# arpg/vicalib

Measured on NVIDIA H100. Metric: lm_iterations_per_sec, higher is better.
Workload: dtype f64

## Files before the change

### vicalib_b200/csrc/vc_imu_math.cuh

```cuda
#pragma once
#include "vc_math.cuh"

namespace vc {
namespace imu {

struct D1 {
  double a, v;
  __host__ __device__ D1() : a(0.0), v(0.0) {}
  __host__ __device__ D1(double s) : a(s), v(0.0) {}
  __host__ __device__ D1(double s, double d) : a(s), v(d) {}
};
__device__ __forceinline__ D1 operator+(D1 x, D1 y) { return {x.a + y.a, x.v + y.v}; }
__device__ __forceinline__ D1 operator-(D1 x, D1 y) { return {x.a - y.a, x.v - y.v}; }
__device__ __forceinline__ D1 operator-(D1 x) { return {-x.a, -x.v}; }
__device__ __forceinline__ D1 operator*(D1 x, D1 y) { return {x.a * y.a, x.a * y.v + x.v * y.a}; }
__device__ __forceinline__ D1 operator/(D1 x, D1 y) {
  const double inv = 1.0 / y.a, q = x.a * inv;
  return {q, (x.v - q * y.v) * inv};
}
__device__ __forceinline__ D1 dsqrt(D1 x) { const double s = sqrt(x.a); return {s, 0.5 * x.v / s}; }
__device__ __forceinline__ double dsqrt(double x) { return sqrt(x); }
__device__ __forceinline__ void dsincos(D1 x, D1* s, D1* c) {
  double sn, cs;
  sincos(x.a, &sn, &cs);
  *s = {sn, cs * x.v};
  *c = {cs, -sn * x.v};
}
__device__ __forceinline__ void dsincos(double x, double* s, double* c) { sincos(x, s, c); }
__device__ __forceinline__ D1 dtan(D1 x) { const double t = tan(x.a); return {t, (1.0 + t * t) * x.v}; }
__device__ __forceinline__ double dtan(double x) { return tan(x); }
__device__ __forceinline__ D1 datan(D1 x) { return {atan(x.a), x.v / (1.0 + x.a * x.a)}; }
__device__ __forceinline__ double datan(double x) { return atan(x); }
__device__ __forceinline__ double val(D1 x) { return x.a; }
__device__ __forceinline__ double val(double x) { return x; }

template <class T> struct Vec { T x, y, z; };
template <class T> struct Quat { T x, y, z, w; };

template <class T> __device__ __forceinline__ Vec<T> operator+(Vec<T> a, Vec<T> b) { return {a.x + b.x, a.y + b.y, a.z + b.z}; }
template <class T> __device__ __forceinline__ Vec<T> operator-(Vec<T> a, Vec<T> b) { return {a.x - b.x, a.y - b.y, a.z - b.z}; }
template <class T> __device__ __forceinline__ Vec<T> scale(Vec<T> a, T s) { return {a.x * s, a.y * s, a.z * s}; }
template <class T> __device__ __forceinline__ Vec<T> cross(Vec<T> a, Vec<T> b) {
  return {a.y * b.z - a.z * b.y, a.z * b.x - a.x * b.z, a.x * b.y - a.y * b.x};
}
template <class T> __device__ __forceinline__ T dot(Vec<T> a, Vec<T> b) { return a.x * b.x + a.y * b.y + a.z * b.z; }

template <class T> __device__ __forceinline__ Quat<T> qmul(Quat<T> a, Quat<T> b) {
  return {a.w * b.x + a.x * b.w + a.y * b.z - a.z * b.y, a.w * b.y + a.y * b.w + a.z * b.x - a.x * b.z,
          a.w * b.z + a.z * b.w + a.x * b.y - a.y * b.x, a.w * b.w - a.x * b.x - a.y * b.y - a.z * b.z};
}
template <class T> __device__ __forceinline__ Quat<T> qconj(Quat<T> q) { return {-q.x, -q.y, -q.z, q.w}; }
template <class T> __device__ __forceinline__ Vec<T> qrot(Quat<T> q, Vec<T> v) {
  const Vec<T> qv{q.x, q.y, q.z};
  Vec<T> uv = cross(qv, v);
  uv = uv + uv;
  return v + scale(uv, q.w) + cross(qv, uv);
}

template <class T> __device__ inline Quat<T> so3_exp(Vec<T> om) {
  const T th2 = dot(om, om);
  T imag, real;
  if (val(th2) < 1e-3) {
    imag = T(0.5) + th2 * (T(-1.0 / 48.0) + th2 * (T(1.0 / 3840.0) + th2 * (T(-1.0 / 645120.0) + th2 * T(1.0 / 185794560.0))));
    real = T(1.0) + th2 * (T(-1.0 / 8.0) + th2 * (T(1.0 / 384.0) + th2 * (T(-1.0 / 46080.0) + th2 * (T(1.0 / 10321920.0) +
                                                                                                   th2 * T(-1.0 / 3715891200.0)))));
  } else {
    const T th = dsqrt(th2);
    T s, c;
    dsincos(th * T(0.5), &s, &c);
    imag = s / th;
    real = c;
  }
  return {imag * om.x, imag * om.y, imag * om.z, real};
}
template <class T> __device__ inline Vec<T> so3_log(Quat<T> q, T* theta) {
  const T n2 = q.x * q.x + q.y * q.y + q.z * q.z;
  T f, n = T(0.0);
  if (val(n2) < kSophusEps * kSophusEps) {
    f = T(2.0) / q.w - T(2.0) * n2 / (q.w * q.w * q.w);
    if (val(n2) > 0.0) n = dsqrt(n2);
  } else {
    n = dsqrt(n2);
    if (fabs(val(q.w)) < kSophusEps) f = T(val(q.w) > 0.0 ? M_PI : -M_PI) / n;
    else f = T(2.0) * datan(n / q.w) / n;
  }
  *theta = f * n;
  return {f * q.x, f * q.y, f * q.z};
}
template <class T> __device__ inline void se3_log(Quat<T> q, Vec<T> t, T out[6]) {
  T th;
  const Vec<T> om = so3_log(q, &th);
  T c;
  if (fabs(val(th)) < kSophusEps) c = T(1.0 / 12.0);
  else c = (T(1.0) - th / (T(2.0) * dtan(th * T(0.5)))) / (th * th);
  const Vec<T> ot = cross(om, t);
  const Vec<T> oot = cross(om, ot);
  const Vec<T> u = t - scale(ot, T(0.5)) + scale(oot, c);
  out[0] = u.x; out[1] = u.y; out[2] = u.z;
  out[3] = om.x; out[4] = om.y; out[5] = om.z;
}

struct ImuBuf {
  const double* d;
  int n;
  double start_time, end_time, average_dt;
};
template <class T> struct Meas { Vec<T> w, a; T time; };

template <class T> __device__ __forceinline__ Meas<T> load_meas(const ImuBuf& b, int i) {
  const int64_t n = b.n;
  return {{T(b.d[n + i]), T(b.d[2 * n + i]), T(b.d[3 * n + i])},
          {T(b.d[4 * n + i]), T(b.d[5 * n + i]), T(b.d[6 * n + i])}, T(b.d[i])};
}
template <class T> __device__ inline Meas<T> interpolate(const ImuBuf& b, int ai, int bi, T ts, double time) {
  const Meas<T> ma = load_meas<T>(b, ai), mb = load_meas<T>(b, bi);
  const T t_a = ma.time + ts, t_b = mb.time + ts, t_out = T(time);
  const T fr = (t_out - t_a) / (t_b - t_a), omf = T(1.0) - fr;
  return {scale(ma.w, omf) + scale(mb.w, fr), scale(ma.a, omf) + scale(mb.a, fr), t_out};
}
template <class T> __device__ inline Meas<T> get_element(const ImuBuf& b, double time, T ts, int* idx) {
  const double off = val(ts);
  const int n = b.n;
  double gd = (time - b.start_time + off) / b.average_dt;
  if (!(gd > 0.0)) gd = 0.0;
  int guess = gd >= static_cast<double>(n) ? n - 1 : static_cast<int>(gd);
  guess = min(guess, n - 1);
  Meas<T> r;
  if (b.d[guess] + off > time) {
    if (guess == 0) {
      r = load_meas<T>(b, 0);
      r.time = r.time + ts;
      *idx = 0;
    } else {
      while ((guess - 1) > 0 && b.d[guess - 1] + off > time) --guess;
      r = interpolate<T>(b, guess - 1, guess, ts, time);
      *idx = guess - 1;
    }
  } else {
    if (guess == n - 1) {
      *idx = guess;
      r = load_meas<T>(b, n - 1);
      r.time = r.time + ts;
    } else {
      while ((guess + 1) < n && (b.d[guess + 1] + off) < time) ++guess;
      r = interpolate<T>(b, guess, guess + 1, ts, time);
      *idx = guess;
    }
  }
  return r;
}
template <class T> __device__ inline bool get_next(const ImuBuf& b, double max_time, T ts, int* idx, Meas<T>* out) {
  if (*idx + 1 >= b.n || b.d[*idx + 1] + val(ts) > max_time) {
    *out = get_element<T>(b, max_time, ts, idx);
    return false;
  }
  *out = load_meas<T>(b, ++*idx);
  out->time = out->time + ts;
  return true;
}

template <class T> struct Pose { Vec<T> p; Quat<T> q; Vec<T> v; };

template <class T> __device__ inline Pose<T> integrate_pose(const Pose<T>& y0, const T k[9], T dt) {
  const Quat<T> dq = so3_exp(Vec<T>{k[3] * dt, k[4] * dt, k[5] * dt});
  Pose<T> y;
  y.p = y0.p + Vec<T>{k[0] * dt, k[1] * dt, k[2] * dt};
  y.q = qmul(dq, y0.q);
  y.v = y0.v + Vec<T>{k[6] * dt, k[7] * dt, k[8] * dt};
  return y;
}
template <class T> __device__ inline void pose_derivative(const Pose<T>& y, Vec<T> g, const Meas<T>& z0, const Meas<T>& z1,
                                                          Vec<T> bg, Vec<T> ba, const T sf[6], T dt, T k[9]) {
  const T alpha = (z1.time - (z0.time + dt)) / (z1.time - z0.time), oma = T(1.0) - alpha;
  const Vec<T> zg = scale(z0.w, alpha) + scale(z1.w, oma);
  const Vec<T> za = scale(z0.a, alpha) + scale(z1.a, oma);
  k[0] = y.v.x; k[1] = y.v.y; k[2] = y.v.z;
  const Vec<T> w = qrot(y.q, Vec<T>{zg.x * sf[0] + bg.x, zg.y * sf[1] + bg.y, zg.z * sf[2] + bg.z});
  k[3] = w.x; k[4] = w.y; k[5] = w.z;
  const Vec<T> a = qrot(y.q, Vec<T>{za.x * sf[3] + ba.x, za.y * sf[4] + ba.y, za.z * sf[5] + ba.z}) - g;
  k[6] = a.x; k[7] = a.y; k[8] = a.z;
}
template <class T> __device__ inline Pose<T> integrate_imu(const Pose<T>& y0, const Meas<T>& z0, const Meas<T>& z1, Vec<T> bg,
                                                           Vec<T> ba, const T sf[6], Vec<T> g) {
  if (val(z1.time) == val(z0.time)) return y0;
  const T dt = z1.time - z0.time;
  T k1[9], k2[9], k3[9], k4[9];
  pose_derivative(y0, g, z0, z1, bg, ba, sf, T(0.0), k1);
  const Pose<T> y1 = integrate_pose(y0, k1, dt * T(0.5));
  pose_derivative(y1, g, z0, z1, bg, ba, sf, dt / T(2.0), k2);
  const Pose<T> y2 = integrate_pose(y0, k2, dt * T(0.5));
  pose_derivative(y2, g, z0, z1, bg, ba, sf, dt / T(2.0), k3);
  const Pose<T> y3 = integrate_pose(y0, k3, dt);
  pose_derivative(y3, g, z0, z1, bg, ba, sf, dt, k4);
#pragma unroll
  for (int i = 0; i < 9; ++i) k1[i] = k1[i] + T(2.0) * k2[i] + T(2.0) * k3[i] + k4[i];
  return integrate_pose(y0, k1, dt / T(6.0));
}

template <class T> __device__ inline Vec<T> gravity_vector(T p, T q) {
  T sp, cp, sq, cq;
  dsincos(p, &sp, &cp);
  dsincos(q, &sq, &cq);
  const T mg = T(-9.8007);
  return {cp * sq * mg, -sp * mg, cp * cq * mg};
}

template <class T>
__device__ inline bool imu_raw_residual(const ImuBuf& buf, double t_start, double t_end, const T x2[7], const T x1[7],
                                        const T v2[3], const T v1[3], const T g2[2], const T b[6], const T sf[6], T ts,
                                        T r[9], Pose<T>* end = nullptr) {
  if (!(t_start >= buf.start_time + val(ts) && t_start <= buf.end_time + val(ts)) || buf.n == 0) return false;
  const Vec<T> g = gravity_vector<T>(g2[0], g2[1]);
  const Vec<T> bg{b[0], b[1], b[2]}, ba{b[3], b[4], b[5]};
  Pose<T> y{{x1[4], x1[5], x1[6]}, {x1[0], x1[1], x1[2], x1[3]}, {v1[0], v1[1], v1[2]}};
  int idx;
  Meas<T> prev = get_element<T>(buf, t_start, ts, &idx), cur;
  bool more = true;
  while (more) {
    more = get_next<T>(buf, t_end, ts, &idx, &cur);
    y = integrate_imu(y, prev, cur, bg, ba, sf, g);
    prev = cur;
  }
  if (end) *end = y;
  const Quat<T> q2i = qconj(Quat<T>{x2[0], x2[1], x2[2], x2[3]});
  const Vec<T> t2i = qrot(q2i, Vec<T>{x2[4], x2[5], x2[6]});
  const Quat<T> qe = qmul(y.q, q2i);
  const Vec<T> te = y.p - qrot(y.q, t2i);
  se3_log(qe, te, r);
  r[6] = y.v.x - v2[0];
  r[7] = y.v.y - v2[1];
  r[8] = y.v.z - v2[2];
  return true;
}

}
}
```

### vicalib_b200/csrc/vc_imu_weights.cuh

```cuda
#pragma once
#include "vc_imu_math.cuh"
#include "vc_internal.h"

namespace vc {
namespace wts {

using imu::Meas;
using imu::Pose;
using imu::Quat;
using imu::Vec;

__device__ inline double powi(double x, int y) {
  double r = x;
  for (int i = 1; i < y; ++i) r *= x;
  return r;
}

__device__ inline void dqx_dq(Quat<double> q, Vec<double> v, double* o, int ld) {
  const double x = v.x, y = v.y, z = v.z;
  const double s1 = 2 * q.x * y, s2 = 2 * q.y * y, s3 = 2 * q.x * x, s4 = 2 * q.z * x, s5 = 2 * q.y * z, s6 = 2 * q.z * z;
  o[0] = s2 + s6; o[1] = s1 - 4 * q.y * x + 2 * q.w * z; o[2] = 2 * q.x * z - 2 * q.w * y - 4 * q.z * x; o[3] = s5 - 2 * q.z * y;
  o[ld + 0] = 2 * q.y * x - 4 * q.x * y - 2 * q.w * z; o[ld + 1] = s3 + s6; o[ld + 2] = s5 + 2 * q.w * x - 4 * q.z * y; o[ld + 3] = s4 - 2 * q.x * z;
  o[2 * ld + 0] = s4 + 2 * q.w * y - 4 * q.x * z; o[2 * ld + 1] = 2 * q.z * y - 2 * q.w * x - 4 * q.y * z; o[2 * ld + 2] = s2 + s3; o[2 * ld + 3] = s1 - 2 * q.y * x;
}
__device__ inline void dq1q2_dq2(Quat<double> q1, double* o, int ld) {
  o[0] = q1.w; o[1] = -q1.z; o[2] = q1.y; o[3] = q1.x;
  o[ld] = q1.z; o[ld + 1] = q1.w; o[ld + 2] = -q1.x; o[ld + 3] = q1.y;
  o[2 * ld] = -q1.y; o[2 * ld + 1] = q1.x; o[2 * ld + 2] = q1.w; o[2 * ld + 3] = q1.z;
  o[3 * ld] = -q1.x; o[3 * ld + 1] = -q1.y; o[3 * ld + 2] = -q1.z; o[3 * ld + 3] = q1.w;
}
__device__ inline void dq1q2_dq1(Quat<double> q2, double* o, int ld) {
  o[0] = q2.w; o[1] = q2.z; o[2] = -q2.y; o[3] = q2.x;
  o[ld] = -q2.z; o[ld + 1] = q2.w; o[ld + 2] = q2.x; o[ld + 3] = q2.y;
  o[2 * ld] = q2.y; o[2 * ld + 1] = -q2.x; o[2 * ld + 2] = q2.w; o[2 * ld + 3] = q2.z;
  o[3 * ld] = -q2.x; o[3 * ld + 1] = -q2.y; o[3 * ld + 2] = -q2.z; o[3 * ld + 3] = q2.w;
}
__device__ inline void dqExp_dw(Vec<double> w, double o[12]) {
  const double t = sqrt(w.x * w.x + w.y * w.y + w.z * w.z);
  const double s1 = t / 20 - 1, s2 = powi(t, 2) / 48 - 0.5;
  const double s3 = (s1 * w.y * w.z) / 24, s4 = (s1 * w.x * w.z) / 24, s5 = (s1 * w.x * w.y) / 24, s6 = powi(t, 2);
  o[0] = (s1 * powi(w.x, 2)) / 24 - s6 / 48 + 0.5; o[1] = s5; o[2] = s4;
  o[3] = s5; o[4] = (s1 * powi(w.y, 2)) / 24 - s6 / 48 + 0.5; o[5] = s3;
  o[6] = s4; o[7] = s3; o[8] = (s1 * powi(w.z, 2)) / 24 - s6 / 48 + 0.5;
  o[9] = (s2 * w.x) / 2; o[10] = (s2 * w.y) / 2; o[11] = (s2 * w.z) / 2;
}
__device__ inline void dLog_dq(Quat<double> q, double o[12]) {
  const double x = q.x, y = q.y, z = q.z, w = q.w;
  const double vsq = powi(x, 2) + powi(y, 2) + powi(z, 2), vn = sqrt(vsq);
  if (vn < 1e-9) {
    const double s1 = 2 * vsq, s2 = 1.0 / powi(w, 3), s3 = (3 * s1) / powi(w, 4) - 2 / powi(w, 2), s4 = 2 / w;
    o[0] = -4 * s2 * powi(x, 2) + s4 - s1 * s2; o[1] = -4 * x * y * s2; o[2] = -4 * x * z * s2; o[3] = x * s3;
    o[4] = -4 * x * y * s2; o[5] = -4 * s2 * powi(y, 2) + s4 - s1 * s2; o[6] = -4 * y * z * s2; o[7] = y * s3;
    o[8] = -4 * x * z * s2; o[9] = -4 * y * z * s2; o[10] = -4 * s2 * powi(z, 2) + s4 - s1 * s2; o[11] = z * s3;
  } else {
    const double s1 = vsq, s2 = 1 / (s1 / powi(w, 2) + 1), s3 = atan(sqrt(s1) / w), s4 = 1 / pow(s1, 1.5), s5 = 1 / s1,
                 s6 = 1 / w, s7 = (2 * s3) / sqrt(s1);
    const double s8 = 2 * y * z * s2 * s5 * s6 - 2 * y * z * s3 * s4;
    const double s9 = 2 * x * z * s2 * s5 * s6 - 2 * x * z * s3 * s4;
    const double s10 = 2 * x * y * s2 * s5 * s6 - 2 * x * y * s3 * s4;
    o[0] = s7 - 2 * powi(x, 2) * s3 * s4 + 2 * powi(x, 2) * s2 * s5 * s6; o[1] = s10; o[2] = s9; o[3] = -(2 * x * s2) / powi(w, 2);
    o[4] = s10; o[5] = s7 - 2 * powi(y, 2) * s3 * s4 + 2 * powi(y, 2) * s2 * s5 * s6; o[6] = s8; o[7] = -(2 * y * s2) / powi(w, 2);
    o[8] = s9; o[9] = s8; o[10] = s7 - 2 * powi(z, 2) * s3 * s4 + 2 * powi(z, 2) * s2 * s5 * s6; o[11] = -(2 * z * s2) / powi(w, 2);
  }
}

__device__ inline void dLog_dSE3(Quat<double> q, Vec<double> tr, double dlog[42]) {
  double dw_dq[12];
  dLog_dq(q, dw_dq);
  const double x = tr.x, y = tr.y, z = tr.z;
  double theta;
  const Vec<double> w = imu::so3_log<double>(q, &theta);
  const double wx = w.x, wy = w.y, wz = w.z;
  const bool close_to_zero = fabs(theta) < kSophusEps;
  const double O[9] = {0, -wz, wy, wz, 0, -wx, -wy, wx, 0};
  double O2[9];
  for (int i = 0; i < 3; ++i)
    for (int j = 0; j < 3; ++j) {
      double s = 0;
      for (int k = 0; k < 3; ++k) s += O[i * 3 + k] * O[k * 3 + j];
      O2[i * 3 + j] = s;
    }
  const double cc = close_to_zero ? 1. / 12. : (1.0 - theta / (2.0 * tan(theta / 2.0))) / (theta * theta);
  for (int i = 0; i < 42; ++i) dlog[i] = 0.0;
  for (int i = 0; i < 3; ++i)
    for (int j = 0; j < 3; ++j) dlog[i * 7 + j] = (i == j ? 1.0 : 0.0) - 0.5 * O[i * 3 + j] + cc * O2[i * 3 + j];
  for (int i = 0; i < 3; ++i)
    for (int j = 0; j < 4; ++j) dlog[(3 + i) * 7 + 3 + j] = dw_dq[i * 4 + j];
  double d[9];
  if (close_to_zero) {
    const double div_12 = 1. / 12, div_6 = 1. / 6.;
    const double wx_x = wx * x, wy_x = wy * x, wz_x = wz * x, wx_y = wx * y, wy_y = wy * y, wz_y = wz * y, wx_z = wx * z,
                 wy_z = wy * z, wz_z = wz * z;
    d[0] = div_12 * (wy_y + wz_z); d[1] = div_12 * wx_y - div_6 * wy_x - 0.5 * z; d[2] = 0.5 * y - div_6 * wz_x + div_12 * wx_z;
    d[3] = 0.5 * z + div_12 * wy_x - div_6 * wx_y; d[4] = div_12 * (wx_x + wz_z); d[5] = div_12 * wy_z - div_6 * wz_y - 0.5 * x;
    d[6] = div_12 * wz_x - div_6 * wx_z - 0.5 * y; d[7] = 0.5 * x + div_12 * wz_y - div_6 * wy_z; d[8] = div_12 * (wx_x * wy_y);
  } else {
    const double s1 = powi(wx, 2) + powi(wy, 2) + powi(wz, 2);
    const double s2 = tan(sqrt(s1) / 2);
    const double s3 = sqrt(s1) / (2 * s2) - 1;
    const double s4 = wz / (2 * sqrt(s1) * s2) - (wz * (powi(s2, 2) + 1)) / (4 * powi(s2, 2));
    const double s5 = wy / (2 * sqrt(s1) * s2) - (wy * (powi(s2, 2) + 1)) / (4 * powi(s2, 2));
    const double s6 = wx / (2 * sqrt(s1) * s2) - (wx * (powi(s2, 2) + 1)) / (4 * powi(s2, 2));
    const double s7 = 1 / s1, s8 = 1 / powi(s1, 2);
    const double s9 = powi(wx, 2) + powi(wy, 2), s10 = powi(wx, 2) + powi(wz, 2), s11 = powi(wy, 2) + powi(wz, 2);
    const double s12 = 2 * s3 * s8 * wx * wy * wz;
    const double s13 = -2 * s3 * s8 * wy * powi(wz, 2) + s4 * s7 * wy * wz + s3 * s7 * wy;
    const double s14 = -2 * s3 * s8 * wx * powi(wz, 2) + s4 * s7 * wx * wz + s3 * s7 * wx;
    const double s15 = -2 * s3 * s8 * wz * powi(wy, 2) + s5 * s7 * wz * wy + s3 * s7 * wz;
    const double s16 = -2 * s3 * s8 * wz * powi(wx, 2) + s6 * s7 * wz * wx + s3 * s7 * wz;
    const double s17 = -2 * s3 * s8 * wx * powi(wy, 2) + s5 * s7 * wx * wy + s3 * s7 * wx;
    const double s18 = -2 * s3 * s8 * wy * powi(wx, 2) + s6 * s7 * wy * wx + s3 * s7 * wy;
    const double s19 = 2 * s3 * s7 * wy, s20 = 2 * s3 * s7 * wx;
    d[0] = x * (s6 * s7 * s11 - 2 * s3 * s8 * s11 * wx) - s18 * y - s16 * z;
    d[1] = x * (s19 + s5 * s7 * s11 - 2 * s3 * s8 * s11 * wy) - s17 * y - z * (s5 * s7 * wx * wz - 2 * s3 * s8 * wx * wy * wz + 0.5);
    d[2] = x * (s4 * s7 * s11 + 2 * s3 * s7 * wz - 2 * s3 * s8 * s11 * wz) - s14 * z + y * (s12 - s4 * s7 * wx * wy + 0.5);
    d[3] = y * (s20 + s6 * s7 * s10 - 2 * s3 * s8 * s10 * wx) - s18 * x + z * (s12 - s6 * s7 * wy * wz + 0.5);
    d[4] = y * (s5 * s7 * s10 - 2 * s3 * s8 * s10 * wy) - s17 * x - s15 * z;
    d[5] = y * (s4 * s7 * s10 + 2 * s3 * s7 * wz - 2 * s3 * s8 * s10 * wz) - s13 * z - x * (s4 * s7 * wx * wy - s12 + 0.5);
    d[6] = z * (s20 + s6 * s7 * s9 - 2 * s3 * s8 * s9 * wx) - s16 * x - y * (s6 * s7 * wy * wz - s12 + 0.5);
    d[7] = z * (s19 + s5 * s7 * s9 - 2 * s3 * s8 * s9 * wy) - s15 * y + x * (s12 - s5 * s7 * wx * wz + 0.5);
    d[8] = z * (s4 * s7 * s9 - 2 * s3 * s8 * s9 * wz) - s14 * x - s13 * y;
  }
  for (int i = 0; i < 3; ++i)
    for (int j = 0; j < 4; ++j) {
      double s = 0;
      for (int k = 0; k < 3; ++k) s += d[i * 3 + k] * dw_dq[k * 4 + j];
      dlog[i * 7 + 3 + j] = s;
    }
}

constexpr int kTeam = 16;
struct Work {
  double C[100], A[100], Gm[60], t1[100], t2[100];
  double rot[8];
  int rpq[8];
};

__device__ __forceinline__ void tmm(double* out, const double* A, const double* B, int R, int K, int C, int tl,
                                    bool transB = false) {
  for (int e = tl; e < R * C; e += kTeam) {
    const int r = e / C, c = e - r * C;
    double s = 0.0;
    for (int k = 0; k < K; ++k) s += A[r * K + k] * (transB ? B[c * K + k] : B[k * C + c]);
    out[e] = s;
  }
}

struct StageJac {
  double R[9];
  double Dw[12];
  double Da[12];
};
__device__ __forceinline__ void stage_jac(const Pose<double>& y, const Meas<double>& z0, const Meas<double>& z1, Vec<double> bg,
                                          Vec<double> ba, double dt, StageJac* J) {
  const double alpha = (z1.time - (z0.time + dt)) / (z1.time - z0.time);
  const Vec<double> zg = imu::scale(z0.w, alpha) + imu::scale(z1.w, 1.0 - alpha);
  const Vec<double> za = imu::scale(z0.a, alpha) + imu::scale(z1.a, 1.0 - alpha);
  qmat(Q4{y.q.x, y.q.y, y.q.z, y.q.w}, J->R);
  dqx_dq(y.q, zg + bg, J->Dw, 4);
  dqx_dq(y.q, za + ba, J->Da, 4);
}
__device__ __forceinline__ void stage_T(const double col[10], int j, const StageJac& J, double T[9]) {
  T[0] = col[7]; T[1] = col[8]; T[2] = col[9];
#pragma unroll
  for (int i = 0; i < 3; ++i) {
    T[3 + i] = J.Dw[i * 4] * col[3] + J.Dw[i * 4 + 1] * col[4] + J.Dw[i * 4 + 2] * col[5] + J.Dw[i * 4 + 3] * col[6];
    T[6 + i] = J.Da[i * 4] * col[3] + J.Da[i * 4 + 1] * col[4] + J.Da[i * 4 + 2] * col[5] + J.Da[i * 4 + 3] * col[6];
  }
  const double sel_g = (j >= 10 && j < 13) ? 1.0 : 0.0, sel_a = j >= 13 ? 1.0 : 0.0;
  const int bc = j >= 13 ? j - 13 : (j >= 10 ? j - 10 : 0);
#pragma unroll
  for (int i = 0; i < 3; ++i) {
    const double rv = bc == 0 ? J.R[i * 3] : (bc == 1 ? J.R[i * 3 + 1] : J.R[i * 3 + 2]);
    T[3 + i] += sel_g * rv;
    T[6 + i] += sel_a * rv;
  }
}
__device__ __forceinline__ Pose<double> integrate_push(const Pose<double>& y0, const double k[9], double h, const double T[9], int j,
                                                       double col[10]) {
  const Vec<double> wdt{k[3] * h, k[4] * h, k[5] * h};
  const Quat<double> r = imu::so3_exp<double>(wdt);
  double a[16], e[12];
  dq1q2_dq1(y0.q, a, 4);
  dqExp_dw(wdt, e);
#pragma unroll
  for (int i = 0; i < 3; ++i) {
    col[i] = h * T[i] + (j == i ? 1.0 : 0.0);
    col[7 + i] = h * T[6 + i] + (j == 7 + i ? 1.0 : 0.0);
  }
  const int jq = j - 3;
  const double Qc[4] = {jq == 0 ? r.w : jq == 1 ? -r.z : jq == 2 ? r.y : r.x,
                        jq == 0 ? r.z : jq == 1 ? r.w : jq == 2 ? -r.x : r.y,
                        jq == 0 ? -r.y : jq == 1 ? r.x : jq == 2 ? r.w : r.z,
                        jq == 0 ? -r.x : jq == 1 ? -r.y : jq == 2 ? -r.z : r.w};
  const bool isq = j >= 3 && j < 7;
#pragma unroll
  for (int i = 0; i < 4; ++i) {
    double s = 0.0;
#pragma unroll
    for (int c = 0; c < 3; ++c) {
      double q = 0.0;
#pragma unroll
      for (int m = 0; m < 4; ++m) q += a[i * 4 + m] * e[m * 3 + c];
      s += q * h * T[3 + c];
    }
    col[3 + i] = s + (isq ? Qc[i] : 0.0);
  }
  return imu::integrate_pose<double>(y0, k, h);
}

__device__ __forceinline__ Pose<double> integrate_imu_cov(const Pose<double>& pose, const Meas<double>& z0, const Meas<double>& z1,
                                                          Vec<double> bg, Vec<double> ba, const double sf[6], Vec<double> g,
                                                          double sg2, double sa2, Work* W, int j, bool on) {
  const double dt = z1.time - z0.time;
  on = on && dt != 0;
  Pose<double> res = pose;
  if (on) {
    double col[10], tot[9], T[9], k1[9], k2[9], k3[9], k4[9];
#pragma unroll
    for (int i = 0; i < 10; ++i) col[i] = (j == i) ? 1.0 : 0.0;
    StageJac J;
    imu::pose_derivative<double>(pose, g, z0, z1, bg, ba, sf, 0.0, k1);
    stage_jac(pose, z0, z1, bg, ba, 0.0, &J);
    stage_T(col, j, J, T);
#pragma unroll
    for (int i = 0; i < 9; ++i) tot[i] = T[i];
    const Pose<double> y1 = integrate_push(pose, k1, dt * 0.5, T, j, col);
    imu::pose_derivative<double>(y1, g, z0, z1, bg, ba, sf, dt / 2, k2);
    stage_jac(y1, z0, z1, bg, ba, dt / 2, &J);
    stage_T(col, j, J, T);
#pragma unroll
    for (int i = 0; i < 9; ++i) tot[i] += 2.0 * T[i];
    const Pose<double> y2 = integrate_push(pose, k2, dt * 0.5, T, j, col);
    imu::pose_derivative<double>(y2, g, z0, z1, bg, ba, sf, dt / 2, k3);
    stage_jac(y2, z0, z1, bg, ba, dt / 2, &J);
    stage_T(col, j, J, T);
#pragma unroll
    for (int i = 0; i < 9; ++i) tot[i] += 2.0 * T[i];
    const Pose<double> y3 = integrate_push(pose, k3, dt, T, j, col);
    imu::pose_derivative<double>(y3, g, z0, z1, bg, ba, sf, dt, k4);
    stage_jac(y3, z0, z1, bg, ba, dt, &J);
    stage_T(col, j, J, T);
#pragma unroll
    for (int i = 0; i < 9; ++i) {
      tot[i] += T[i];
      k1[i] = k1[i] + 2 * k2[i] + 2 * k3[i] + k4[i];
    }
    res = integrate_push(pose, k1, dt / 6.0, tot, j, col);
    if (j < 10) {
#pragma unroll
      for (int i = 0; i < 10; ++i) W->A[i * 10 + j] = col[i];
    } else {
#pragma unroll
      for (int i = 0; i < 10; ++i) W->Gm[i * 6 + (j - 10)] = col[i];
    }
  }
  __syncwarp();
  if (on) tmm(W->t1, W->A, W->C, 10, 10, 10, j);
  __syncwarp();
  if (on) tmm(W->t2, W->t1, W->A, 10, 10, 10, j, true);
  __syncwarp();
  if (on)
    for (int e = j; e < 100; e += kTeam) {
      const int r = e / 10, c = e - r * 10;
      double s = 0.0;
#pragma unroll
      for (int q = 0; q < 6; ++q) s += W->Gm[r * 6 + q] * (q < 3 ? sg2 : sa2) * W->Gm[c * 6 + q];
      W->C[e] = W->t2[e] + s;
    }
  __syncwarp();
  return res;
}

struct WeightArgs {
  DevProblem dp;
  imu::ImuBuf buf;
  const Ctl* ctl;
  const double* states[2];
  const double* ftime;
  double* wsqrt;
  int ni;
  double sigma_g, sigma_a;
  int deferred;
};
constexpr int kWtWarps = 4;
constexpr int kWtTeams = kWtWarps * (32 / kTeam);

__device__ __forceinline__ void weight_from_cov(const Pose<double>& y, const double* X2, Work* W, int tl, bool on, double* out,
                                                double* vec) {
  const Quat<double> q2i = imu::qconj(Quat<double>{X2[0], X2[1], X2[2], X2[3]});
  const Vec<double> t2 = imu::qrot(q2i, Vec<double>{X2[4], X2[5], X2[6]});
  const Vec<double> t2i{-t2.x, -t2.y, -t2.z};
  const Quat<double> q12 = imu::qmul(y.q, q2i);
  const Vec<double> t12 = y.p + imu::qrot(y.q, t2i);
  double* dlog = W->t1;
  double* dmul = W->t1 + 42;
  double* Jt = W->t2;
  if (on) {
    for (int e = tl; e < 49; e += kTeam) dmul[e] = (e % 8 == 0 && e < 3 * 8) ? 1.0 : 0.0;
    for (int e = tl; e < 90; e += kTeam) Jt[e] = (e == 67 || e == 78 || e == 89) ? 1.0 : 0.0;
  }
  __syncwarp();
  if (on && tl == 0) dLog_dSE3(q12, t12, dlog);
  if (on && tl == 1) {
    dqx_dq(y.q, t2i, dmul + 3, 7);
    dq1q2_dq1(q2i, dmul + 3 * 7 + 3, 7);
  }
  __syncwarp();
  if (on)
    for (int e = tl; e < 42; e += kTeam) {
      const int i = e / 7, jj = e - i * 7;
      double s = 0.0;
#pragma unroll
      for (int q = 0; q < 7; ++q) s += dlog[i * 7 + q] * dmul[q * 7 + jj];
      Jt[i * 10 + jj] = s;
    }
  __syncwarp();
  if (on) tmm(W->t1, Jt, W->C, 9, 10, 10, tl);
  __syncwarp();
  double* A = W->A;
  double* V = W->C;
  if (on) tmm(A, W->t1, Jt, 9, 10, 9, tl, true);
  __syncwarp();
  bool cold = false;
  if (on)
    for (int e = tl; e < 81; e += kTeam) {
      const double v = vec[e];
      cold = cold || v != v;
      V[e] = v;
    }
  cold = ((__ballot_sync(0xffffffffu, cold) >> (threadIdx.x & 16)) & 0xffffu) != 0;
  if (on && cold)
    for (int e = tl; e < 81; e += kTeam) V[e] = (e % 10 == 0) ? 1.0 : 0.0;
  __syncwarp();
  if (on)
    for (int e = tl; e < 81; e += kTeam) {
      const int r = e / 9, c = e - r * 9;
      double s = 0.0;
      for (int k = 0; k < 9; ++k) s += 0.5 * (A[r * 9 + k] + A[k * 9 + r]) * V[k * 9 + c];
      W->t1[e] = s;
    }
  __syncwarp();
  if (on)
    for (int e = tl; e < 81; e += kTeam) {
      const int r = e / 9, c = e - r * 9;
      if (c >= r) {
        double s = 0.0;
        for (int k = 0; k < 9; ++k) s += V[k * 9 + r] * W->t1[k * 9 + c];
        W->t2[r * 9 + c] = s;
        W->t2[c * 9 + r] = s;
      }
    }
  __syncwarp();
  A = W->t2;
  for (int sweep = 0; sweep < 40; ++sweep) {
    double off = 0.0, dg = 0.0;
    if (on) {
#pragma unroll
      for (int i = 0; i < 9; ++i) {
        dg += A[i * 9 + i] * A[i * 9 + i];
#pragma unroll
        for (int jj = i + 1; jj < 9; ++jj) off += A[i * 9 + jj] * A[i * 9 + jj];
      }
    }
    const bool conv = !on || off <= 1e-30 * dg;
    if (__all_sync(0xffffffffu, conv)) break;
    for (int r = 0; r < 9; ++r) {
      if (on && !conv && tl < 4) {
        int cnt = 0, pi = 0, qi = 0;
#pragma unroll
        for (int i = 0; i < 9; ++i) {
          const int jj = (r - i + 9) % 9;
          if (i < jj) {
            if (cnt == tl) { pi = i; qi = jj; }
            ++cnt;
          }
        }
        const double apq = A[pi * 9 + qi];
        double c = 1.0, sn = 0.0;
        if (apq != 0.0) {
          const double tau = (A[qi * 9 + qi] - A[pi * 9 + pi]) / (2.0 * apq);
          const double t = (tau >= 0 ? 1.0 : -1.0) / (fabs(tau) + sqrt(1.0 + tau * tau));
          c = rsqrt(1.0 + t * t);
          sn = t * c;
        }
        W->rot[2 * tl] = c; W->rot[2 * tl + 1] = sn;
        W->rpq[2 * tl] = pi; W->rpq[2 * tl + 1] = qi;
      }
      __syncwarp();
      if (on && !conv)
        for (int e = tl; e < 36; e += kTeam) {
          const int k = e >> 2, t = e & 3, p = W->rpq[2 * t], q = W->rpq[2 * t + 1];
          const double c = W->rot[2 * t], sn = W->rot[2 * t + 1];
          const double akp = A[k * 9 + p], akq = A[k * 9 + q];
          A[k * 9 + p] = c * akp - sn * akq;
          A[k * 9 + q] = sn * akp + c * akq;
          const double vkp = V[k * 9 + p], vkq = V[k * 9 + q];
          V[k * 9 + p] = c * vkp - sn * vkq;
          V[k * 9 + q] = sn * vkp + c * vkq;
        }
      __syncwarp();
      if (on && !conv)
        for (int e = tl; e < 36; e += kTeam) {
          const int k = e >> 2, t = e & 3, p = W->rpq[2 * t], q = W->rpq[2 * t + 1];
          const double c = W->rot[2 * t], sn = W->rot[2 * t + 1];
          const double apk = A[p * 9 + k], aqk = A[q * 9 + k];
          A[p * 9 + k] = c * apk - sn * aqk;
          A[q * 9 + k] = sn * apk + c * aqk;
        }
      __syncwarp();
    }
  }
  if (!on) return;
  for (int e = tl; e < 81; e += kTeam) vec[e] = V[e];
  bool singular = false;
#pragma unroll
  for (int k = 0; k < 9; ++k) singular = singular || !(A[k * 9 + k] > 0.0);
  if (singular) return;
  if (tl < 9) W->t1[tl] = 1.0 / sqrt(A[tl * 9 + tl]);
  __syncwarp(0xffffu << (threadIdx.x & 16));
  for (int e = tl; e < 81; e += kTeam) {
    const int r = e / 9, c = e - r * 9;
    double s = 0.0;
#pragma unroll
    for (int k = 0; k < 9; ++k) s += V[r * 9 + k] * W->t1[k] * V[c * 9 + k];
    out[e] = s;
  }
}

template <class A>
__device__ __forceinline__ void imu_weights_team(const A& a, const double* state, int kk, Work* W, int tl) {
  const int ki = min(kk, a.ni - 1);
  const double* X1 = state + 7 * static_cast<int64_t>(ki);
  const double* X2 = state + 7 * static_cast<int64_t>(ki + 1);
  const double* V1 = state + a.dp.off_v + 3 * static_cast<int64_t>(ki);
  const double* P = state + a.dp.off_imu;
  const double ts = P[14];
  const double t_start = a.ftime[ki], t_end = a.ftime[ki + 1];
  bool on = kk < a.ni && (t_start >= a.buf.start_time + ts && t_start <= a.buf.end_time + ts) && a.buf.n > 0;
  const Vec<double> g = imu::gravity_vector<double>(P[0], P[1]);
  const Vec<double> bg{P[2], P[3], P[4]}, ba{P[5], P[6], P[7]};
  double sf[6];
#pragma unroll
  for (int i = 0; i < 6; ++i) sf[i] = P[8 + i];
  Pose<double> y{{X1[4], X1[5], X1[6]}, {X1[0], X1[1], X1[2], X1[3]}, {V1[0], V1[1], V1[2]}};
  __syncwarp();
  for (int e = tl; e < 100; e += kTeam) W->C[e] = 0.0;
  __syncwarp();
  const double sg2 = a.sigma_g * a.sigma_g, sa2 = a.sigma_a * a.sigma_a;
  int idx = 0;
  Meas<double> prev{}, cur{};
  if (on) prev = imu::get_element<double>(a.buf, t_start, ts, &idx);
  bool more = on;
  while (__any_sync(0xffffffffu, more)) {
    const bool step = more;
    if (step) more = imu::get_next<double>(a.buf, t_end, ts, &idx, &cur);
    y = integrate_imu_cov(y, prev, cur, bg, ba, sf, g, sg2, sa2, W, tl, step);
    if (step) prev = cur;
  }
  weight_from_cov(y, X2, W, tl, on, a.wsqrt + static_cast<int64_t>(ki) * 81, a.wsqrt + static_cast<int64_t>(a.ni + ki) * 81);
}

__global__ void __launch_bounds__(32 * kWtWarps, 2) imu_weights_kernel(WeightArgs a) {
  __shared__ Work work[kWtTeams];
  const int tl = threadIdx.x & (kTeam - 1);
  const int team = threadIdx.x / kTeam;
  if (a.deferred) {
    if (!(a.ctl->iter > 0 && a.ctl->last_accepted)) return;
  } else {
    if (a.ctl->done) return;
    if (a.ctl->iter > 0 && !a.ctl->last_accepted) return;
  }
  if (blockIdx.x * kWtTeams + (threadIdx.x >> 5) * (32 / kTeam) >= a.ni) return;
  imu_weights_team(a, a.states[a.ctl->cur], blockIdx.x * kWtTeams + team, &work[team], tl);
}

}
}
```

Measured before the change: 2015.

## Reuse interpolated IMU measurements and rotation, restructure covariance propagation per column

Interpolated gyro/accel values are now computed once per RK stage time and shared between the derivative and the Jacobian; the two middle stages share one interpolation. The so3_exp already computed in integrate_push is passed into integrate_pose instead of being recomputed. Divisions by constants are replaced with multiplications by reciprocals. The A*C*A^T + G*Q*G^T covariance update becomes a column-per-lane register-accumulated computation with one fewer warp sync, leaving lanes j>=10 idle, and a trailing syncwarp is added before the weight computation.

```diff
diff --git a/vicalib_b200/csrc/vc_imu_math.cuh b/vicalib_b200/csrc/vc_imu_math.cuh
--- a/vicalib_b200/csrc/vc_imu_math.cuh
+++ b/vicalib_b200/csrc/vc_imu_math.cuh
@@ -161,24 +161,34 @@
 
 template <class T> struct Pose { Vec<T> p; Quat<T> q; Vec<T> v; };
 
-template <class T> __device__ inline Pose<T> integrate_pose(const Pose<T>& y0, const T k[9], T dt) {
-  const Quat<T> dq = so3_exp(Vec<T>{k[3] * dt, k[4] * dt, k[5] * dt});
+template <class T> __device__ inline Pose<T> integrate_pose(const Pose<T>& y0, const T k[9], T dt, Quat<T> dq) {
   Pose<T> y;
   y.p = y0.p + Vec<T>{k[0] * dt, k[1] * dt, k[2] * dt};
   y.q = qmul(dq, y0.q);
   y.v = y0.v + Vec<T>{k[6] * dt, k[7] * dt, k[8] * dt};
   return y;
 }
-template <class T> __device__ inline void pose_derivative(const Pose<T>& y, Vec<T> g, const Meas<T>& z0, const Meas<T>& z1,
-                                                          Vec<T> bg, Vec<T> ba, const T sf[6], T dt, T k[9]) {
+template <class T> __device__ inline Pose<T> integrate_pose(const Pose<T>& y0, const T k[9], T dt) {
+  return integrate_pose(y0, k, dt, so3_exp(Vec<T>{k[3] * dt, k[4] * dt, k[5] * dt}));
+}
+template <class T> __device__ inline void interp_meas(const Meas<T>& z0, const Meas<T>& z1, T dt, Vec<T>* zg, Vec<T>* za) {
   const T alpha = (z1.time - (z0.time + dt)) / (z1.time - z0.time), oma = T(1.0) - alpha;
-  const Vec<T> zg = scale(z0.w, alpha) + scale(z1.w, oma);
-  const Vec<T> za = scale(z0.a, alpha) + scale(z1.a, oma);
+  *zg = scale(z0.w, alpha) + scale(z1.w, oma);
+  *za = scale(z0.a, alpha) + scale(z1.a, oma);
+}
+template <class T> __device__ inline void pose_derivative_at(const Pose<T>& y, Vec<T> g, Vec<T> zg, Vec<T> za, Vec<T> bg, Vec<T> ba,
+                                                             const T sf[6], T k[9]) {
   k[0] = y.v.x; k[1] = y.v.y; k[2] = y.v.z;
   const Vec<T> w = qrot(y.q, Vec<T>{zg.x * sf[0] + bg.x, zg.y * sf[1] + bg.y, zg.z * sf[2] + bg.z});
   k[3] = w.x; k[4] = w.y; k[5] = w.z;
   const Vec<T> a = qrot(y.q, Vec<T>{za.x * sf[3] + ba.x, za.y * sf[4] + ba.y, za.z * sf[5] + ba.z}) - g;
   k[6] = a.x; k[7] = a.y; k[8] = a.z;
+}
+template <class T> __device__ inline void pose_derivative(const Pose<T>& y, Vec<T> g, const Meas<T>& z0, const Meas<T>& z1,
+                                                          Vec<T> bg, Vec<T> ba, const T sf[6], T dt, T k[9]) {
+  Vec<T> zg, za;
+  interp_meas(z0, z1, dt, &zg, &za);
+  pose_derivative_at(y, g, zg, za, bg, ba, sf, k);
 }
 template <class T> __device__ inline Pose<T> integrate_imu(const Pose<T>& y0, const Meas<T>& z0, const Meas<T>& z1, Vec<T> bg,
                                                            Vec<T> ba, const T sf[6], Vec<T> g) {
diff --git a/vicalib_b200/csrc/vc_imu_weights.cuh b/vicalib_b200/csrc/vc_imu_weights.cuh
--- a/vicalib_b200/csrc/vc_imu_weights.cuh
+++ b/vicalib_b200/csrc/vc_imu_weights.cuh
@@ -36,13 +36,14 @@
   o[3 * ld] = -q2.x; o[3 * ld + 1] = -q2.y; o[3 * ld + 2] = -q2.z; o[3 * ld + 3] = q2.w;
 }
 __device__ inline void dqExp_dw(Vec<double> w, double o[12]) {
+  constexpr double r20 = 1.0 / 20, r24 = 1.0 / 24, r48 = 1.0 / 48;
   const double t = sqrt(w.x * w.x + w.y * w.y + w.z * w.z);
-  const double s1 = t / 20 - 1, s2 = powi(t, 2) / 48 - 0.5;
-  const double s3 = (s1 * w.y * w.z) / 24, s4 = (s1 * w.x * w.z) / 24, s5 = (s1 * w.x * w.y) / 24, s6 = powi(t, 2);
-  o[0] = (s1 * powi(w.x, 2)) / 24 - s6 / 48 + 0.5; o[1] = s5; o[2] = s4;
-  o[3] = s5; o[4] = (s1 * powi(w.y, 2)) / 24 - s6 / 48 + 0.5; o[5] = s3;
-  o[6] = s4; o[7] = s3; o[8] = (s1 * powi(w.z, 2)) / 24 - s6 / 48 + 0.5;
-  o[9] = (s2 * w.x) / 2; o[10] = (s2 * w.y) / 2; o[11] = (s2 * w.z) / 2;
+  const double s1 = t * r20 - 1, s2 = powi(t, 2) * r48 - 0.5;
+  const double s3 = (s1 * w.y * w.z) * r24, s4 = (s1 * w.x * w.z) * r24, s5 = (s1 * w.x * w.y) * r24, s6 = powi(t, 2);
+  o[0] = (s1 * powi(w.x, 2)) * r24 - s6 * r48 + 0.5; o[1] = s5; o[2] = s4;
+  o[3] = s5; o[4] = (s1 * powi(w.y, 2)) * r24 - s6 * r48 + 0.5; o[5] = s3;
+  o[6] = s4; o[7] = s3; o[8] = (s1 * powi(w.z, 2)) * r24 - s6 * r48 + 0.5;
+  o[9] = (s2 * w.x) * 0.5; o[10] = (s2 * w.y) * 0.5; o[11] = (s2 * w.z) * 0.5;
 }
 __device__ inline void dLog_dq(Quat<double> q, double o[12]) {
   const double x = q.x, y = q.y, z = q.z, w = q.w;
@@ -151,11 +152,8 @@
   double Dw[12];
   double Da[12];
 };
-__device__ __forceinline__ void stage_jac(const Pose<double>& y, const Meas<double>& z0, const Meas<double>& z1, Vec<double> bg,
-                                          Vec<double> ba, double dt, StageJac* J) {
-  const double alpha = (z1.time - (z0.time + dt)) / (z1.time - z0.time);
-  const Vec<double> zg = imu::scale(z0.w, alpha) + imu::scale(z1.w, 1.0 - alpha);
-  const Vec<double> za = imu::scale(z0.a, alpha) + imu::scale(z1.a, 1.0 - alpha);
+__device__ __forceinline__ void stage_jac(const Pose<double>& y, Vec<double> zg, Vec<double> za, Vec<double> bg, Vec<double> ba,
+                                          StageJac* J) {
   qmat(Q4{y.q.x, y.q.y, y.q.z, y.q.w}, J->R);
   dqx_dq(y.q, zg + bg, J->Dw, 4);
   dqx_dq(y.q, za + ba, J->Da, 4);
@@ -206,7 +204,7 @@
     }
     col[3 + i] = s + (isq ? Qc[i] : 0.0);
   }
-  return imu::integrate_pose<double>(y0, k, h);
+  return imu::integrate_pose<double>(y0, k, h, r);
 }
 
 __device__ __forceinline__ Pose<double> integrate_imu_cov(const Pose<double>& pose, const Meas<double>& z0, const Meas<double>& z1,
@@ -220,26 +218,30 @@
 #pragma unroll
     for (int i = 0; i < 10; ++i) col[i] = (j == i) ? 1.0 : 0.0;
     StageJac J;
-    imu::pose_derivative<double>(pose, g, z0, z1, bg, ba, sf, 0.0, k1);
-    stage_jac(pose, z0, z1, bg, ba, 0.0, &J);
+    Vec<double> zg, za;
+    imu::interp_meas<double>(z0, z1, 0.0, &zg, &za);
+    imu::pose_derivative_at<double>(pose, g, zg, za, bg, ba, sf, k1);
+    stage_jac(pose, zg, za, bg, ba, &J);
     stage_T(col, j, J, T);
 #pragma unroll
     for (int i = 0; i < 9; ++i) tot[i] = T[i];
     const Pose<double> y1 = integrate_push(pose, k1, dt * 0.5, T, j, col);
-    imu::pose_derivative<double>(y1, g, z0, z1, bg, ba, sf, dt / 2, k2);
-    stage_jac(y1, z0, z1, bg, ba, dt / 2, &J);
+    imu::interp_meas<double>(z0, z1, dt / 2, &zg, &za);
+    imu::pose_derivative_at<double>(y1, g, zg, za, bg, ba, sf, k2);
+    stage_jac(y1, zg, za, bg, ba, &J);
     stage_T(col, j, J, T);
 #pragma unroll
     for (int i = 0; i < 9; ++i) tot[i] += 2.0 * T[i];
     const Pose<double> y2 = integrate_push(pose, k2, dt * 0.5, T, j, col);
-    imu::pose_derivative<double>(y2, g, z0, z1, bg, ba, sf, dt / 2, k3);
-    stage_jac(y2, z0, z1, bg, ba, dt / 2, &J);
+    imu::pose_derivative_at<double>(y2, g, zg, za, bg, ba, sf, k3);
+    stage_jac(y2, zg, za, bg, ba, &J);
     stage_T(col, j, J, T);
 #pragma unroll
     for (int i = 0; i < 9; ++i) tot[i] += 2.0 * T[i];
     const Pose<double> y3 = integrate_push(pose, k3, dt, T, j, col);
-    imu::pose_derivative<double>(y3, g, z0, z1, bg, ba, sf, dt, k4);
-    stage_jac(y3, z0, z1, bg, ba, dt, &J);
+    imu::interp_meas<double>(z0, z1, dt, &zg, &za);
+    imu::pose_derivative_at<double>(y3, g, zg, za, bg, ba, sf, k4);
+    stage_jac(y3, zg, za, bg, ba, &J);
     stage_T(col, j, J, T);
 #pragma unroll
     for (int i = 0; i < 9; ++i) {
@@ -256,19 +258,41 @@
     }
   }
   __syncwarp();
-  if (on) tmm(W->t1, W->A, W->C, 10, 10, 10, j);
-  __syncwarp();
-  if (on) tmm(W->t2, W->t1, W->A, 10, 10, 10, j, true);
-  __syncwarp();
-  if (on)
-    for (int e = j; e < 100; e += kTeam) {
-      const int r = e / 10, c = e - r * 10;
+  if (on && j < 10) {
+    double m[10], cc[10];
+#pragma unroll
+    for (int k = 0; k < 10; ++k) cc[k] = W->C[k * 10 + j];
+#pragma unroll
+    for (int r = 0; r < 10; ++r) m[r] = 0.0;
+#pragma unroll
+    for (int k = 0; k < 10; ++k)
+#pragma unroll
+      for (int r = 0; r < 10; ++r) m[r] += W->A[r * 10 + k] * cc[k];
+#pragma unroll
+    for (int r = 0; r < 10; ++r) W->t1[r * 10 + j] = m[r];
+#pragma unroll
+    for (int r = 0; r < 10; ++r) {
       double s = 0.0;
 #pragma unroll
-      for (int q = 0; q < 6; ++q) s += W->Gm[r * 6 + q] * (q < 3 ? sg2 : sa2) * W->Gm[c * 6 + q];
-      W->C[e] = W->t2[e] + s;
-    }
-  __syncwarp();
+      for (int q = 0; q < 6; ++q) s += W->Gm[r * 6 + q] * (q < 3 ? sg2 : sa2) * W->Gm[j * 6 + q];
+      W->C[r * 10 + j] = s;
+      W->t2[r * 10 + j] = W->A[j * 10 + r];
+    }
+  }
+  __syncwarp();
+  if (on && j < 10) {
+    double c2[10];
+#pragma unroll
+    for (int r = 0; r < 10; ++r) c2[r] = 0.0;
+#pragma unroll
+    for (int k = 0; k < 10; ++k) {
+      const double a = W->t2[k * 10 + j];
+#pragma unroll
+      for (int r = 0; r < 10; ++r) c2[r] += W->t1[r * 10 + k] * a;
+    }
+#pragma unroll
+    for (int r = 0; r < 10; ++r) W->C[r * 10 + j] = c2[r] + W->C[r * 10 + j];
+  }
   return res;
 }
 
@@ -458,6 +482,7 @@
     y = integrate_imu_cov(y, prev, cur, bg, ba, sf, g, sg2, sa2, W, tl, step);
     if (step) prev = cur;
   }
+  __syncwarp();
   weight_from_cov(y, X2, W, tl, on, a.wsqrt + static_cast<int64_t>(ki) * 81, a.wsqrt + static_cast<int64_t>(a.ni + ki) * 81);
 }
 
```

New measurement: 2018, median of 6. No clear change (+0.2%).
